# CITlabRostock/citlab-article-separation-new

Measured on AMD Instinct MI355X. Metric: newspaper pages/sec (ARU-Net seg + GNN relation) at 3000x4500 px, higher is better.
Workload: dtype f32s

## Files before the change

### citlab-article-separation-new_amd/csrc/aru_engine.hip

```cpp
#include <algorithm>
#include <cmath>
#include <cstdlib>
#include <memory>

#include "aru_kernels.h"
#include "res8_kernels.h"
#include "res8v_kernels.h"
#include "bf16_kernels.h"
#include "res8w_kernels.h"
#include "res8ws_kernels.h"
#include "level0_plan.h"
#include "launch_plan.h"
#include "convr_kernels.h"
#include "split_kernels.h"
#include "pyr_kernels.h"
#include "asep_common.h"
#include "aru_pack.h"

using namespace asep;

namespace {

struct Tensor {
    float* p = nullptr;
    int H = 0, W = 0, C = 0;
    bool bf = false;
    size_t count() const { return (size_t)H * W * C; }
    bf16_t* bp() const { return reinterpret_cast<bf16_t*>(p); }
};

struct PackedConv : ConvPlan {
    float* d_w = nullptr;
    float* d_b = nullptr;
    float* d_wino = nullptr;
    float* d_wv = nullptr;
    bf16_t* d_wb = nullptr;
    bf16_t* d_wb8 = nullptr;
    bf16_t* d_ws = nullptr;
    bf16_t* d_ws16 = nullptr;
};

struct DirectConv {
    int k = 0, cout = 0, cin = 1;
    float* d_w = nullptr;
    float* d_b = nullptr;
};

}

struct asep_aru {
    asep_aru_cfg cfg{};
    std::map<std::string, PackedConv> convs;
    struct ResB { int C = 0; bf16_t* d_w = nullptr; float* d_b = nullptr; };
    std::map<std::string, ResB> resb;
    std::map<std::string, float*> taps;
    bf16_t* d_r8b_down_w = nullptr;
    float* d_r8b_down_b = nullptr;
    bf16_t* d_r8b_up_w1 = nullptr;
    bf16_t* d_r8f_up_w1 = nullptr;
    bf16_t* d_r8f_down_w1 = nullptr;
    float* d_r8b_down_w1r = nullptr;
    bool use_res32 = true;
    int walk_mode = 1;
    bool use_deconvs = true;
    bool use_convr = true;
    unsigned char* d_zero_trash = nullptr;
    int fused_act = 0;
    bool use_walk = true;
    bf16_t* d_r8b_up_w = nullptr;
    float* d_r8b_up_b = nullptr;
    float* d_r8b_up_b1 = nullptr;
    DirectConv det_first, att_first;
    float* d_r8_down_wr = nullptr;
    float* d_r8_down_br = nullptr;
    float* d_r8_up_w1 = nullptr;
    float* d_r8_up_wr = nullptr;
    float* d_r8_up_br = nullptr;
    float* d_r8_up_b1 = nullptr;
    float* d_r8v_down_wr = nullptr;
    float* d_r8v_up_w1 = nullptr;
    float* d_r8v_up_wr = nullptr;
    bool r8_valu = true;
    bool use_split_walk = true;
    bf16_t* d_r8ws_down_w = nullptr;
    bf16_t* d_r8ws_up_w = nullptr;
    bf16_t* d_r8ws_up_w1 = nullptr;
    bool use_fused8 = true;
    bool fused8_wanted = true;
    bool fused8_var = false;
    float* d_att_head = nullptr;
    bf16_t* d_att_headb = nullptr;
    float* d_logit_w = nullptr;
    float* d_logit_b = nullptr;
    float* d_logit_wd = nullptr;
    float* d_stats = nullptr;
    const float* const* page_stats = nullptr;
    double* d_sums = nullptr;
    struct Lane {
        hipStream_t s = nullptr;
        bool own_stream = false;
        hipStream_t side = nullptr;
        hipEvent_t ev_fork = nullptr, ev_join = nullptr, ev_begin = nullptr, ev_done = nullptr;
        hipStream_t bside = nullptr;
        hipEvent_t ev_bfork = nullptr, ev_bjoin = nullptr;
        BufferPool pool;
        ~Lane() {
            if (ev_fork) (void)hipEventDestroy(ev_fork);
            if (ev_bfork) (void)hipEventDestroy(ev_bfork);
            if (ev_bjoin) (void)hipEventDestroy(ev_bjoin);
            if (ev_join) (void)hipEventDestroy(ev_join);
            if (ev_begin) (void)hipEventDestroy(ev_begin);
            if (ev_done) (void)hipEventDestroy(ev_done);
            if (side) (void)hipStreamDestroy(side);
            if (bside) (void)hipStreamDestroy(bside);
            if (own_stream && s) (void)hipStreamDestroy(s);
        }
    };
    std::vector<std::unique_ptr<Lane>> lanes;
    Lane* cur = nullptr;
    int last_nl = 0;
    bool lanes_forced = false;
    int num_lanes = 2;
    std::map<std::string, Tensor> endpoints;
    hipStream_t stream = nullptr;
    std::vector<void*> owned;

    struct ProfRec { int kid; double flops, bytes, xflops; hipEvent_t a, b; };
    int num_cus = 256;
    BufferPool host_stage;
    hipStream_t host_stream = nullptr;
    bool use_xcd_sched = true;
    std::map<std::string, const int32_t*> sched_cache;
    bool bf16 = false;
    bool split = false;
    bool use_c12 = true;
    bool fuse_pool = true;
    bool fuse_act = true;
    bool profiling = false;
    bool prof_detail = false;
    bool prof_in_situ = false;
    std::vector<std::string> prof_names;
    std::vector<ProfRec> prof_recs;
    std::vector<hipEvent_t> ev_pool;
    size_t ev_next = 0;

    ~asep_aru() {
        for (void* p : owned)
            if (p) (void)hipFree(p);
        for (hipEvent_t e : ev_pool) (void)hipEventDestroy(e);
        if (host_stream) (void)hipStreamDestroy(host_stream);
    }
    hipEvent_t next_event() {
        if (ev_next == ev_pool.size()) {
            hipEvent_t e;
            ASEP_HIP_CHECK_THROW(hipEventCreate(&e));
            ev_pool.push_back(e);
        }
        return ev_pool[ev_next++];
    }
    int prof_kid(const std::string& name) {
        for (size_t i = 0; i < prof_names.size(); ++i)
            if (prof_names[i] == name) return (int)i;
        prof_names.push_back(name);
        return (int)prof_names.size() - 1;
    }
    int feat(int l) const { return cfg.feat_root << l; }
// ... 414 lines not shown
        ProfScope ps(m, name, 0.0);
        ps.bytes = k.bytes;
        launch(a, dim3(k.units.total));
    });
}

TL run_pool(asep_aru* m, const TL& in, PoolKind kind) {
    TL out;
    for (const Tensor& t : in) {
        if (kind == POOL_CHANSUM) out.push_back(new_tensor(m, t.H, t.W, 1));
        else out.push_back(new_tensor(m, cdiv(t.H, 2), cdiv(t.W, 2), t.C));
    }
    stream_pass<PoolArgs>(m, in, kind == POOL_MAX ? "maxpool2_kernel" : (kind == POOL_AVG_C1 ? "avgpool2_c1_kernel" : (kind == POOL_AVG_C3 ? "avgpool2_cn_kernel<3>" : "chansum_kernel")), POOL_ITEMS,
        [&](PoolProb& p, size_t i, Chunk& k) {
            k.bytes += tbytes(in[i]) + tbytes(out[i]);
            p.in = in[i].p; p.out = out[i].p; p.H = in[i].H; p.W = in[i].W; p.Ho = out[i].H; p.Wo = out[i].W;
            return kind == POOL_MAX ? out[i].count() / 4 : (size_t)out[i].H * out[i].W;
        }, [&](const PoolArgs& a, dim3 grid) {
            if (kind == POOL_MAX) hipLaunchKernelGGL(maxpool2_kernel, grid, dim3(256), 0, m->stream, a);
            else if (kind == POOL_AVG_C1) hipLaunchKernelGGL(avgpool2_c1_kernel, grid, dim3(256), 0, m->stream, a);
            else if (kind == POOL_AVG_C3) launch_avgpool_c3(m, a, grid);
            else hipLaunchKernelGGL(chansum_kernel, grid, dim3(256), 0, m->stream, a);
        });
    return out;
}

int grid_1d(size_t n) { return (int)std::min<size_t>((n + 255) / 256, 256 * 8); }

std::string res8_what(bool up, const TL& l) {
    return (up ? "unet_up_0 (conv1[16->8]+3xconvR+add) " : "unet_down_0 (conv1+3xconvR+add+pool) ") + dims_of(l);
}

bool r8v_fits(const TL& l) {
    for (const Tensor& t : l)
        if ((size_t)t.H * t.W >= ((size_t)1 << 28)) return false;
    return true;
}

bool r8ws_fits(const Tensor& t) { return walk_region(t.H, t.W).fits; }
bool r8ws_on(asep_aru* m) { return m->split && m->use_split_walk && m->r8_valu && m->cfg.activation == 0 && m->d_r8ws_down_w; }
const int32_t* r8ws_frame_units(asep_aru* m, const Res8Args& a, const std::vector<bool>& walk, int* count) {
    std::string key = "f";
    for (int i = 0; i < a.nprob; ++i) key += ":" + std::to_string(a.p[i].H) + "x" + std::to_string(a.p[i].W) + (walk[i] ? "w" : "t");
    std::vector<int32_t> units;
    for (int i = 0; i < a.nprob; ++i) frame_units(a.p[i].H, a.p[i].W, a.p[i].tiles_x, a.p[i].tile_begin, walk[i], R8_OW, R8_OH * R8_NP, &units);
    *count = (int)units.size();
    auto it = m->sched_cache.find(key);
    if (it != m->sched_cache.end()) return it->second;
    if (units.empty()) return nullptr;
    const int32_t* d = put_table(m, units);
    if (d) m->sched_cache[key] = d;
    return d;
}

void run_res8ws(asep_aru* m, bool up, const Res8Args& a, const std::vector<bool>& walk, const std::string& what) {
    Res8WSArgs wa{};
    int n = 0, items = 0;
    double flops = 0, bytes = 0;
    long strip_rows = 0;
    for (int i = 0; i < a.nprob; ++i) {
        if (!walk[i]) continue;
        const Res8Prob& q = a.p[i];
        Res8WSProb& p = wa.p[n++];
        if (up) { p.skip = q.img; p.dec = q.in1; }
        else { p.img = q.img; p.stats = q.stats; p.pool = q.pool; }
        p.out = q.out;
        p.H = q.H; p.W = q.W;
        const WalkRegion r = walk_region(p.H, p.W);
        p.n_strips = r.n_strips;
        p.y_end = r.y_end;
        strip_rows += (long)r.n_strips * r.rows();
        flops += 2.0 * r.pixels() * (9.0 * (up ? 16 : 1) * 8 + 3 * 9.0 * 64);
        bytes += r.pixels() * ((up ? 64.0 : 4.0) + 32.0 + (p.pool ? 8.0 : 0.0));
    }
    if (!n) return;
    const int band = walk_band(strip_rows, m->num_cus, 4);
    for (int i = 0; i < n; ++i) {
        Res8WSProb& p = wa.p[i];
        p.band = band;
        p.tile_begin = items;
        items += walk_region(p.H, p.W).items(band);
    }
    wa.nprob = n;
    if (up) { wa.b1 = m->d_r8_up_b1; wa.w1s = (const u32x4*)m->d_r8ws_up_w1; wa.ws = (const u32x4*)m->d_r8ws_up_w; wa.bias = m->d_r8_up_br; }
    else { wa.b1 = m->det_first.d_b; wa.w1f = m->det_first.d_w; wa.ws = (const u32x4*)m->d_r8ws_down_w; wa.bias = m->d_r8_down_br; }
    int units = items;
    wa.xm = oneshot_map(m, items, &units);
    ProfScope ps(m, up ? "res8ws_kernel<true>" : "res8ws_kernel<false>", flops, what);
    ps.bytes = bytes;
    if (up) hipLaunchKernelGGL(res8ws_kernel<true>, dim3(units), dim3(64), 0, m->stream, wa);
    else hipLaunchKernelGGL(res8ws_kernel<false>, dim3(units), dim3(64), 0, m->stream, wa);
}

struct Res8Kernel { void (*fn)(const Res8Args); const char* name; };
Res8Kernel res8_kernel(bool up, bool valu, int actv) {
    static const Res8Kernel k[2][4] = {
        {{res8v_down_kernel<0>, "res8v_down_kernel<0>"}, {res8v_down_kernel<1>, "res8v_down_kernel<1>"}, {res8v_down_kernel<2>, "res8v_down_kernel<2>"},
         {res8_down_kernel<false>, "res8_down_kernel<false>"}},
        {{res8v_up_kernel<0>, "res8v_up_kernel<0>"}, {res8v_up_kernel<1>, "res8v_up_kernel<1>"}, {res8v_up_kernel<2>, "res8v_up_kernel<2>"},
         {res8_up_kernel<false>, "res8_up_kernel<false>"}}};
    return k[up][valu ? actv : 3];
}

void run_res8(asep_aru* m, bool up, const TL& in0, const TL* in1, const std::vector<const float*>& stats, bool want_pool, TL* d_out, TL* pool_out) {
    for (const Tensor& t : in0) {
        d_out->push_back(new_tensor(m, t.H, t.W, 8));
        if (want_pool) pool_out->push_back(new_tensor(m, cdiv(t.H, 2), cdiv(t.W, 2), 8));
    }
    const size_t lds = up ? R8_UP_LDS : R8_DOWN_LDS;
    const char* layer = up ? "unet_up_0" : "unet_down_0";
    for_chunks<Res8Args>(in0.size(), 0.0, [&](Res8Prob& p, size_t i, Chunk& k) {
        k.bytes += tbytes(in0[i]) + (up ? tbytes((*in1)[i]) : 0.0) + tbytes((*d_out)[i]) + (want_pool ? tbytes((*pool_out)[i]) : 0.0);
        p.img = in0[i].p; p.in1 = up ? (*in1)[i].p : nullptr; p.stats = stats.empty() ? nullptr : stats[i];
        p.out = (*d_out)[i].p; p.pool = want_pool ? (*pool_out)[i].p : nullptr;
        p.H = in0[i].H; p.W = in0[i].W;
        set_tiles(p, k.units.next_tiles(p.H, p.W, R8_OW, R8_OH * R8_NP));
        k.flops += 2.0 * in0[i].H * in0[i].W * (9.0 * (up ? 16 : 1) * 8 + 3 * 9.0 * 64);
    }, [&](Res8Args& a, const Chunk& c) {
        const int tiles = c.units.total;
        const double flops = c.flops, bytes = c.bytes;
        const TL sub = c.sub(in0);
        const bool valu = m->r8_valu && r8v_fits(sub);
        if (up) { a.w1 = valu ? m->d_r8v_up_w1 : m->d_r8_up_w1; a.b1 = m->d_r8_up_b1; }
        else { a.w1 = m->det_first.d_w; a.b1 = m->det_first.d_b; }
        a.wr = (const f32x4*)(up ? (valu ? m->d_r8v_up_wr : m->d_r8_up_wr) : (valu ? m->d_r8v_down_wr : m->d_r8_down_wr));
        a.br = up ? m->d_r8_up_br : m->d_r8_down_br;
        const int actv = m->cfg.activation;
        const Res8Kernel k = res8_kernel(up, valu, actv);
        a.sched = tile_schedule(m, a, std::min(tiles, m->num_cus), R8_OH * R8_NP);
        if (valu && r8ws_on(m) && (!up || m->d_r8ws_up_w1)) {
            std::vector<bool> walk(a.nprob);
            bool any = false;
            for (int i = 0; i < a.nprob; ++i) { walk[i] = r8ws_fits(sub[i]); any = any || walk[i]; }
            if (any) {
                int nu = 0;
                Res8Args f = a;
                f.sched = r8ws_frame_units(m, a, walk, &nu);
                if (!f.sched) { set_error("level-0 frame schedule: device allocation failed"); throw ArgError(); }
                f.total_tiles = nu;
                {
                    const double share = (double)nu / tiles;
                    ProfScope ps(m, k.name, flops * share, std::string(layer) + " frame " + dims_of(sub));
                    ps.bytes = bytes * share;
                    hipLaunchKernelGGL(k.fn, dim3(std::min(nu, m->num_cus)), dim3(R8_THREADS), lds, m->stream, f);
                }
                run_res8ws(m, up, a, walk, res8_what(up, sub));
                return;
            }
        }
        ProfScope ps(m, k.name, flops, res8_what(up, sub));
        ps.bytes = bytes;
        if (actv && !valu) { set_error("level-0 block of an elu / leaky graph: image too large for the vector-ALU kernel"); throw ArgError(); }
        hipLaunchKernelGGL(k.fn, dim3(std::min(tiles, m->num_cus)), dim3(R8_THREADS), lds, m->stream, a);
    });
}

void run_res8b_tiles(asep_aru* m, bool up, const TL& a0, const TL* a1, const std::vector<const float*>& stats, bool want_pool, const TL& outs, const TL* pool_out);

void run_res8w(asep_aru* m, bool up, const TL& in0, const TL* dec, const std::vector<const float*>& stats, const TL& outs, const TL* pools) {
    for (size_t c = 0; c < num_chunks(in0.size()); ++c) {
        const size_t b0 = chunk_begin(c), b1 = chunk_end(in0.size(), c);
        Res8WArgs wa{};
        Res8WBArgs ba{};
        double flops = 0, bytes = 0, wshare = 0;
        long strip_rows = 0;
        for (size_t i = b0; i < b1; ++i) {
// ... 915 lines not shown
    }
    if (fusedb && cfg->res_depth == 3)
        for (int l = 0; l < n; ++l) {
            const int f = cfg->feat_root << l;
            if (f != 8 && f != 16 && !(f == 32 && m->use_res32)) continue;
            for (const char* side : {"down", "up"}) {
                if (side[0] == 'u' && l == n - 1) continue;
                const std::string scope = std::string("aru_net/featMapG/unet_") + side + "_" + std::to_string(l);
                const ResbPack p = pack_resb(blob, scope, f);
                if (p.ok) m->resb[scope] = {f, m->put(p.w), m->put(p.b)};
            }
        }
    const Layer logit = find_layer(blob, "aru_net/logit/class");
    if (!has_shape(logit.w, 4, 4, cfg->feat_root, cfg->n_classes)) {
        set_error("weights: aru_net/logit/class/weights must be [4,4,%d,%d]", cfg->feat_root, cfg->n_classes);
        throw PackRefusal{ASEP_ERR_WEIGHTS};
    }
    m->d_logit_w = m->put(logit.w.data);
    m->d_logit_b = m->put(logit.b.data);
    if (cfg->n_classes == 2) m->d_logit_wd = m->put(pack_logit_diff(logit));
}

}

extern "C" {

asep_aru* asep_aru_load(const void* weight_blob, size_t nbytes, const asep_aru_cfg* cfg) {
    ASEP_GUARD_BEGIN
    if (!cfg || !weight_blob) { set_error("asep_aru_load: null argument"); return nullptr; }
    if (cfg->struct_size != (int32_t)sizeof(asep_aru_cfg)) {
        set_error("asep_aru_load: cfg.struct_size is %d, this library's asep_aru_cfg has %zu bytes (ABI version %d): the binding was "
                  "written against another include/asep_hip.h", cfg->struct_size, sizeof(asep_aru_cfg), ASEP_ABI_VERSION);
        return nullptr;
    }
    if (cfg->channels != 1 && cfg->channels != 3) { set_error("asep_aru_load: %d input channels: 1 (gray) and 3 (RGB) are supported", cfg->channels); return nullptr; }
    if (cfg->channels == 3 && cfg->use_attention) {
        set_error("asep_aru_load: 3-channel input needs a graph without attention (RU or U): the attention graph upsamples its attention map to the "
                  "input's shape with a one-channel filter (ARU_v1.py:115)");
        return nullptr;
    }
    if (cfg->compute_dtype < 0 || cfg->compute_dtype > 2) { set_error("asep_aru_load: compute_dtype %d unknown (0 = fp32, 1 = bf16 MFMA, 2 = fp32 with split bf16 products)", cfg->compute_dtype); return nullptr; }
    if (cfg->scale_space_num < 1 || cfg->res_depth < 1) { set_error("asep_aru_load: bad cfg"); return nullptr; }
    if (cfg->activation < 0 || cfg->activation > 2) { set_error("asep_aru_load: activation %d unknown (0 = relu, 1 = elu, 2 = leaky)", cfg->activation); return nullptr; }
    const bool variant = cfg->activation != 0 || cfg->plain_u != 0;
    if (cfg->plain_u && cfg->use_attention) { set_error("asep_aru_load: graph 'U' has no attention branch (ARU_v1.py:92-97)"); return nullptr; }
    if (cfg->inp4up && !cfg->input_pyramid) { set_error("asep_aru_load: inp4up is an option of the input-pyramid graph (RU_v2.py:143): set input_pyramid"); return nullptr; }
    if (cfg->input_pyramid && (cfg->use_attention || cfg->plain_u)) {
        set_error("asep_aru_load: the input-pyramid graph (RU_v2) is a residual U-Net without attention (RU_v2.py:56: useResidual=True, no attMapG): "
                  "use_attention and plain_u must be 0");
        return nullptr;
    }
    if (cfg->input_pyramid && cfg->compute_dtype == 1) {
        set_error("asep_aru_load: the input-pyramid graph (RU_v2) is served by the fp32 engines (compute_dtype 0 or 2): the bf16 engine's fused block "
                  "tails round conv1's result to bfloat16 before the pooled page's term could be added");
        return nullptr;
    }
    std::map<std::string, HostTensor> blob;
    if (!parse_blob(weight_blob, nbytes, blob)) return nullptr;
    std::map<std::string, std::vector<float>> taps;
    if (cfg->input_pyramid) {
        try {
            blob = split_pyramid_blob(blob, *cfg, taps);
        } catch (const PackRefusal&) {
            return nullptr;
        }
    }
    warn_ignored_switches();
    std::unique_ptr<asep_aru> m(new asep_aru());
    m->cfg = *cfg;
    m->bf16 = cfg->compute_dtype == 1;
    m->split = cfg->compute_dtype == 2;
    if (const char* e = getenv("ASEP_FUSE_POOL")) m->fuse_pool = atoi(e) != 0;
    if (const char* e = getenv("ASEP_FUSE_ACT")) m->fuse_act = atoi(e) != 0;
    if (const char* e = getenv("ASEP_C12")) m->use_c12 = atoi(e) != 0;
    if (const char* e = getenv("ASEP_FUSED8")) m->use_fused8 = atoi(e) != 0;
    m->fused8_wanted = m->use_fused8;
    if (variant) m->use_fused8 = false;
    if (const char* e = getenv("ASEP_R8_VALU")) m->r8_valu = atoi(e) != 0;
    m->fused8_var = variant && !cfg->plain_u && cfg->activation != 0 && m->fused8_wanted && m->r8_valu && m->fuse_act && !m->bf16;
    if (const char* e = getenv("ASEP_XCD_SCHED")) m->use_xcd_sched = atoi(e) != 0;
    if (const char* e = getenv("ASEP_BF_RES32")) m->use_res32 = atoi(e) != 0;
    if (const char* e = getenv("ASEP_BF_CONVR")) m->use_convr = atoi(e) != 0;
    if (const char* e = getenv("ASEP_SPLIT_DECONV")) m->use_deconvs = atoi(e) != 0;
    if (const char* e = getenv("ASEP_SPLIT_WALK")) m->use_split_walk = atoi(e) != 0;
    if (const char* e = getenv("ASEP_BF_WALK")) { m->walk_mode = atoi(e); m->use_walk = m->walk_mode != 0; }
    if (const char* e = getenv("ASEP_LANES")) { m->num_lanes = std::max(1, std::min(4, atoi(e))); m->lanes_forced = true; }
    for (int l = 0; l < m->num_lanes; ++l) {
        std::unique_ptr<asep_aru::Lane> L(new asep_aru::Lane());
        bool ok = hipStreamCreateWithFlags(&L->side, hipStreamNonBlocking) == hipSuccess &&
                  hipStreamCreateWithFlags(&L->bside, hipStreamNonBlocking) == hipSuccess &&
                  hipEventCreateWithFlags(&L->ev_fork, hipEventDisableTiming) == hipSuccess &&
                  hipEventCreateWithFlags(&L->ev_bfork, hipEventDisableTiming) == hipSuccess &&
                  hipEventCreateWithFlags(&L->ev_bjoin, hipEventDisableTiming) == hipSuccess &&
                  hipEventCreateWithFlags(&L->ev_join, hipEventDisableTiming) == hipSuccess &&
                  hipEventCreateWithFlags(&L->ev_begin, hipEventDisableTiming) == hipSuccess &&
                  hipEventCreateWithFlags(&L->ev_done, hipEventDisableTiming) == hipSuccess;
        if (ok && l > 0) { ok = hipStreamCreateWithFlags(&L->s, hipStreamNonBlocking) == hipSuccess; L->own_stream = ok; }
        if (!ok) { set_error("asep_aru_load: cannot create streams/events for lane %d", l); return nullptr; }
        m->lanes.push_back(std::move(L));
    }
    m->cur = m->lanes[0].get();
    for (const auto& t : taps) m->taps[t.first] = m->put(t.second);
    try {
        load_weights(m.get(), blob, variant);
    } catch (const PackRefusal&) {
        return nullptr;
    }
    {
        hipDeviceProp_t prop;
        int dev = 0;
        if (hipGetDevice(&dev) == hipSuccess && hipGetDeviceProperties(&prop, dev) == hipSuccess && prop.multiProcessorCount > 0)
            m->num_cus = prop.multiProcessorCount;
    }
    m->d_stats = m->alloc<float>(2);
    m->d_sums = m->alloc<double>(2);
    m->d_zero_trash = m->alloc<unsigned char>(8192);
    ASEP_HIP_CHECK_THROW(hipMemset(m->d_zero_trash, 0, 8192));
    return m.release();
    ASEP_GUARD_END_PTR
}

void asep_aru_free(asep_aru* m) { delete m; }

static int forward_lanes(asep_aru* m, int n_pages, const float* const* d_imgs, const int32_t* Hs, const int32_t* Ws, float* const* d_outs,
                         uint8_t* const* d_u8, uint8_t* const* d_mask, float threshold, hipStream_t stream) {
    m->endpoints.clear();
    const int by_pages = m->lanes_forced ? n_pages : n_pages / 4;
    const int nl = (m->profiling || n_pages < 2) ? 1 : std::max(1, std::min<int>((int)m->lanes.size(), by_pages));
    asep_aru::Lane& L0 = *m->lanes[0];
    L0.s = stream;
    if (nl != m->last_nl && n_pages > 1) {
        if (m->last_nl != 0)
            for (auto& Lp : m->lanes) Lp->pool.release();
        m->last_nl = nl;
    }
    if (nl == 1) return forward_impl(m, L0, 0, n_pages, d_imgs, Hs, Ws, d_outs, d_u8, d_mask, threshold);
    ASEP_HIP_CHECK(hipEventRecord(L0.ev_begin, stream));
    int page0 = 0;
    for (int l = 0; l < nl; ++l) {
        asep_aru::Lane& L = *m->lanes[l];
        const int cnt = n_pages / nl + (l < n_pages % nl ? 1 : 0);
        if (l > 0) ASEP_HIP_CHECK(hipStreamWaitEvent(L.s, L0.ev_begin, 0));
        int rc = forward_impl(m, L, page0, cnt, d_imgs + page0, Hs + page0, Ws + page0, d_outs + page0, d_u8 ? d_u8 + page0 : nullptr,
                              d_mask ? d_mask + page0 : nullptr, threshold);
        if (rc) return rc;
        if (l > 0) {
            ASEP_HIP_CHECK(hipEventRecord(L.ev_done, L.s));
            ASEP_HIP_CHECK(hipStreamWaitEvent(stream, L.ev_done, 0));
        }
        page0 += cnt;
    }
    m->stream = stream;
    return ASEP_OK;
}

int asep_aru_forward_dev(asep_aru* m, const float* d_img, int H, int W, float* d_out, uint8_t* d_out_u8,
                         uint8_t* d_out_mask, float threshold, void* stream) {
    ASEP_GUARD_BEGIN
    if (!m || !d_img || !d_out || H < 1 || W < 1) { set_error("asep_aru_forward_dev: bad argument"); return ASEP_ERR_ARG; }
    const int32_t h1 = H, w1 = W;
    return forward_lanes(m, 1, &d_img, &h1, &w1, &d_out, d_out_u8 ? &d_out_u8 : nullptr, d_out_mask ? &d_out_mask : nullptr,
                         threshold, (hipStream_t)stream);
    ASEP_GUARD_END
}

int asep_aru_forward_batch_dev(asep_aru* m, int n_pages, const float* const* d_imgs, int H, int W, float* const* d_outs,
                               uint8_t* const* d_out_u8, uint8_t* const* d_out_mask, float threshold, void* stream) {
// ... 180 lines not shown
```

### citlab-article-separation-new_amd/csrc/res8ws_kernels.h

```cpp
#pragma once
#include "res8w_kernels.h"
#include "split_kernels.h"

namespace asep {

struct Res8WSProb {
    const float* skip;
    const float* dec;
    const float* img;
    const float* stats;
    float* out;
    float* pool;
    int H, W;
    int n_strips;
    int band;
    int y_end;
    int tile_begin;
};
struct Res8WSArgs {
    Res8WSProb p[MAXP];
    int nprob;
    const float* b1;
    const u32x4* w1s;
    const float* w1f;
    const u32x4* ws;
    const float* bias;
    XcdMap xm;
};

__device__ __forceinline__ void r8ws_mm6(const u32x4 (&w)[3], const u32x4 (&xa)[3], const u32x4 (&xb)[3], f32x4& ca, f32x4& cb) {
    ca = mfma_bf16_k32(w[2], xa[0], ca); cb = mfma_bf16_k32(w[2], xb[0], cb);
    ca = mfma_bf16_k32(w[0], xa[2], ca); cb = mfma_bf16_k32(w[0], xb[2], cb);
    ca = mfma_bf16_k32(w[1], xa[1], ca); cb = mfma_bf16_k32(w[1], xb[1], cb);
    ca = mfma_bf16_k32(w[1], xa[0], ca); cb = mfma_bf16_k32(w[1], xb[0], cb);
    ca = mfma_bf16_k32(w[0], xa[1], ca); cb = mfma_bf16_k32(w[0], xb[1], cb);
    ca = mfma_bf16_k32(w[0], xa[0], ca); cb = mfma_bf16_k32(w[0], xb[0], cb);
}
__device__ __forceinline__ void r8ws_split4(f32x4 v, u32x2& h, u32x2& m, u32x2& l) {
    unsigned h0, m0, l0, h1, m1, l1;
    split3_pair(v.x, v.y, h0, m0, l0);
    split3_pair(v.z, v.w, h1, m1, l1);
    h = u32x2{h0, h1}; m = u32x2{m0, m1}; l = u32x2{l0, l1};
}

template <bool UP>
__global__ __launch_bounds__(64, 1) void res8ws_kernel(const Res8WSArgs a) {
    constexpr int TW = R8W_TW;
    constexpr int W0 = TW + 6, W1 = TW + 4, W2 = TW + 2;
    constexpr int NR = 4, NT = 16;
    constexpr int PL0 = W0 * 16, PL1 = W1 * 16, PL2 = W2 * 16;
    constexpr int IMB = UP ? 0 : 4 * 32 * 4;
    constexpr int R0_OFF = IMB, R1_OFF = R0_OFF + NR * 3 * PL0, R2_OFF = R1_OFF + NR * 3 * PL1, TC_OFF = R2_OFF + NR * 3 * PL2,
                  TRASH = TC_OFF + NT * TW * 32, LDSB = TRASH + 16;
    static_assert(LDSB <= 30 * 1024, "four waves per CU with room to spare");
    __shared__ __attribute__((aligned(16))) unsigned char lds[LDSB];

    const int lane = threadIdx.x;
    const int j = lane & 15, kk = lane >> 4, e = kk >> 1, ch = (kk & 1) * 4;
    const int isB = kk & 1;
    const int c = 2 * j + e;
    const int item = sched_tile(a.xm);
    if (item < 0) return;
    const int pi = prob_of_tile(a, item);
    const Res8WSProb& P = a.p[pi];
    const int li = item - P.tile_begin;
    const int bi = li / P.n_strips, si = li - bi * P.n_strips;
    const int x0 = R8W_X0 + TW * si;
    const int Ya = R8W_Y0 + bi * P.band;
    const int nb = min(P.band, P.y_end - Ya);
    const int W = P.W;

    constexpr int NF1 = UP ? 18 : 0, NFW = 27;
    u32x4 wf[NFW], w1[UP ? NF1 : 1];
    {
        const u32x4* wl = a.ws + lane;
#pragma unroll
        for (int i = 0; i < NFW; ++i) asm volatile("global_load_dwordx4 %0, %1, off" : "=a"(wf[i]) : "v"(wl + i * 64) : "memory");
        if constexpr (UP) {
            const u32x4* w1l = a.w1s + lane;
#pragma unroll
            for (int i = 0; i < NF1; ++i) asm volatile("global_load_dwordx4 %0, %1, off" : "=a"(w1[i]) : "v"(w1l + i * 64) : "memory");
        }
        asm volatile("s_waitcnt vmcnt(0)" ::: "memory");
#pragma unroll
        for (int i = 0; i < NFW; ++i) asm volatile("" : "+a"(wf[i]));
        if constexpr (UP) {
#pragma unroll
            for (int i = 0; i < NF1; ++i) asm volatile("" : "+a"(w1[i]));
        }
    }
    auto wpart = [&](int s, int ky, u32x4 (&o)[3]) {
#pragma unroll
        for (int p = 0; p < 3; ++p) o[p] = wf[(s * 3 + ky) * 3 + p];
    };
    const f32x4 bias1 = *reinterpret_cast<const f32x4*>(a.b1 + ch);
    f32x4 biasw[3];
#pragma unroll
    for (int t = 0; t < 3; ++t) biasw[t] = *reinterpret_cast<const f32x4*>(a.bias + 8 * t + ch);

    const int gxw = min(x0 - 4 + 2 * j + kk, W - 1);
    const float* __restrict__ skp = P.skip;
    const float* __restrict__ dcp = P.dec;
    auto in_row = [&](const float* __restrict__ src, int gy, f32x4& lo, f32x4& hi) {
        const float* q = src + ((size_t)gy * (size_t)W + (size_t)gxw) * 8;
        lo = *reinterpret_cast<const f32x4*>(q);
        hi = *reinterpret_cast<const f32x4*>(q + 4);
    };
    float mean = 0.f, inv = 1.f;
    if constexpr (!UP) {
        if (P.stats) { mean = P.stats[0]; inv = P.stats[1]; }
    }
    const float* __restrict__ imp = P.img;
    const size_t ioff0 = (size_t)(Ya - 4 + (lane >> 5)) * (size_t)W + (size_t)(x0 - 4 + (lane & 31));
    auto iload = [&](int p) { return imp[ioff0 + (size_t)p * 2 * (size_t)W]; };
    float* const iring = reinterpret_cast<float*>(lds);
    auto istore = [&](float v, int p) { iring[(p & 1) * 64 + lane] = (v - mean) * inv; };
    float w1v[UP ? 1 : 36];
    if constexpr (!UP) {
#pragma unroll
        for (int t = 0; t < 9; ++t)
#pragma unroll
            for (int o = 0; o < 4; ++o) w1v[t * 4 + o] = a.w1f[t * 8 + ch + o];
    }

    const int p_last = nb / 2 + 3;
    u32x4 cin[2][2][3] = {};
    f32x4 nxt[2][2][2];
    float inx = 0.f;
    if constexpr (UP) {
#pragma unroll
        for (int r = 0; r < 2; ++r) {
            f32x4 lo, hi;
            in_row(skp, Ya - 4 + r, lo, hi);
            split3_x8(lo, hi, cin[r][0][0], cin[r][0][1], cin[r][0][2]);
            in_row(dcp, Ya - 4 + r, lo, hi);
            split3_x8(lo, hi, cin[r][1][0], cin[r][1][1], cin[r][1][2]);
            in_row(skp, Ya - 2 + r, nxt[r][0][0], nxt[r][0][1]);
            in_row(dcp, Ya - 2 + r, nxt[r][1][0], nxt[r][1][1]);
        }
    } else {
        istore(iload(0), 0);
        inx = iload(1);
    }

    const int lcol = r8w_swz(2 * j + kk) * 16;
    auto whole = [&](u32x2 pa, u32x2 pb) {
        const auto s0 = __builtin_amdgcn_permlane16_swap(pa.x, pb.x, false, false);
        const auto s1 = __builtin_amdgcn_permlane16_swap(pa.y, pb.y, false, false);
        return u32x4{s0[0], s1[0], s0[1], s1[1]};
    };
    const int cs = r8w_swz(c) * 16;
    const bool v0 = j < W0 / 2, v1 = j < W1 / 2, v2 = j < W2 / 2;
    const bool tvalid = c >= 3 && c < 3 + TW;
    const int tcol = (tvalid ? c - 3 : 0) * 32 + ch * 4;
    const int trd = min(c, TW - 1) * 32 + ch * 4;
    const bool ost = j < TW / 2;
    float* __restrict__ const outp = P.out;
    float* __restrict__ const poolp = P.pool;
    const size_t Wp = (size_t)((W + 1) >> 1);

    auto store_parts = [&](f32x4 ra, f32x4 rb, int roff, int pl, bool valid, int rowa, int rowb) {
        u32x2 ha, ma, la, hb, mb, lb;
        r8ws_split4(relu4i(ra), ha, ma, la);
        r8ws_split4(relu4i(rb), hb, mb, lb);
        const u32x4 ph = whole(ha, hb), pm = whole(ma, mb), pl_ = whole(la, lb);
        const int rr = isB ? rowb : rowa;
        const int base = valid ? roff + rr * 3 * pl + cs : TRASH;
        const int step = valid ? pl : 0;
        *reinterpret_cast<u32x4*>(lds + base) = ph;
        *reinterpret_cast<u32x4*>(lds + base + step) = pm;
        *reinterpret_cast<u32x4*>(lds + base + 2 * step) = pl_;
    };
    auto ring_read = [&](int roff, int pl, int rr, u32x4 (&o)[3]) {
#pragma unroll
        for (int p = 0; p < 3; ++p) o[p] = *reinterpret_cast<const u32x4*>(lds + roff + (rr * 3 + p) * pl + lcol);
    };

    const int K = nb / 2 + 6;
#pragma unroll 1
    for (int k = 0; k < K; ++k) {
        const int i4 = (2 * k) & (NR - 1), i16 = (2 * k) & (NT - 1);
        const bool do_c1 = k < nb / 2 + 3, do_s1 = k >= 2 && k < nb / 2 + 4, do_s2 = k >= 4 && k < nb / 2 + 5, do_s3 = k >= 6;

        if (do_s3) {
            u32x4 q[4][3];
#pragma unroll
            for (int r = 0; r < 4; ++r) ring_read(R2_OFF, PL2, (i4 + r - 9) & (NR - 1), q[r]);
            const f32x4 t0 = *reinterpret_cast<const f32x4*>(lds + TC_OFF + ((i16 - 8) & (NT - 1)) * TW * 32 + trd);
            const f32x4 t1 = *reinterpret_cast<const f32x4*>(lds + TC_OFF + ((i16 - 7) & (NT - 1)) * TW * 32 + trd);
            f32x4 va = biasw[2], vb = biasw[2];
#pragma unroll
            for (int ky = 0; ky < 3; ++ky) {
                u32x4 w[3];
                wpart(2, ky, w);
                r8ws_mm6(w, q[ky], q[ky + 1], va, vb);
            }
            va = relu4i(va + t0);
            vb = relu4i(vb + t1);
            const int oy = Ya - 12 + 2 * k;
            if (ost) {
                float* o = outp + ((size_t)oy * (size_t)W + (size_t)(x0 + c)) * 8 + ch;
                *reinterpret_cast<f32x4*>(o) = va;
                *reinterpret_cast<f32x4*>(o + (size_t)W * 8) = vb;
            }
            if constexpr (!UP) {
                if (poolp) {
                    const f32x4 mv = f32x4{fmaxf(va.x, vb.x), fmaxf(va.y, vb.y), fmaxf(va.z, vb.z), fmaxf(va.w, vb.w)};
                    float pm[4];
#pragma unroll
                    for (int i = 0; i < 4; ++i) {
                        const unsigned u = __float_as_uint(mv[i]);
                        const auto s = __builtin_amdgcn_permlane32_swap(u, u, false, false);
                        pm[i] = fmaxf(__uint_as_float(s[0]), __uint_as_float(s[1]));
                    }
                    if (ost && e == 0) {
                        float* po = poolp + ((size_t)(oy >> 1) * Wp + (size_t)((x0 >> 1) + j)) * 8 + ch;
                        *reinterpret_cast<f32x4*>(po) = f32x4{pm[0], pm[1], pm[2], pm[3]};
                    }
                }
            }
        }
        if (do_s2) {
            u32x4 q[4][3];
#pragma unroll
            for (int r = 0; r < 4; ++r) ring_read(R1_OFF, PL1, (i4 + r - 6) & (NR - 1), q[r]);
            f32x4 ra = biasw[1], rb = biasw[1];
#pragma unroll
            for (int ky = 0; ky < 3; ++ky) {
                u32x4 w[3];
                wpart(1, ky, w);
                r8ws_mm6(w, q[ky], q[ky + 1], ra, rb);
            }
            store_parts(ra, rb, R2_OFF, PL2, v2, (i4 - 5) & (NR - 1), (i4 - 4) & (NR - 1));
        }
        if (do_s1) {
            u32x4 q[4][3];
#pragma unroll
            for (int r = 0; r < 4; ++r) ring_read(R0_OFF, PL0, (i4 + r - 3) & (NR - 1), q[r]);
            f32x4 ra = biasw[0], rb = biasw[0];
#pragma unroll
            for (int ky = 0; ky < 3; ++ky) {
                u32x4 w[3];
                wpart(0, ky, w);
                r8ws_mm6(w, q[ky], q[ky + 1], ra, rb);
            }
            store_parts(ra, rb, R1_OFF, PL1, v1, (i4 - 2) & (NR - 1), (i4 - 1) & (NR - 1));
        }
        if (do_c1) {
            f32x4 ra = bias1, rb = bias1;
            if constexpr (UP) {
                u32x4 x2[2][2][3];
#pragma unroll
                for (int r = 0; r < 2; ++r)
#pragma unroll
                    for (int s = 0; s < 2; ++s) split3_x8(nxt[r][s][0], nxt[r][s][1], x2[r][s][0], x2[r][s][1], x2[r][s][2]);
                if (k + 2 <= p_last) {
#pragma unroll
                    for (int r = 0; r < 2; ++r) {
                        in_row(skp, Ya + 2 * k + r, nxt[r][0][0], nxt[r][0][1]);
                        in_row(dcp, Ya + 2 * k + r, nxt[r][1][0], nxt[r][1][1]);
                    }
                }
#pragma unroll
                for (int ky = 0; ky < 3; ++ky)
#pragma unroll
                    for (int s = 0; s < 2; ++s) {
                        u32x4 w[3];
#pragma unroll
                        for (int p = 0; p < 3; ++p) w[p] = w1[(ky * 2 + s) * 3 + p];
                        u32x4 xa[3], xb[3];
#pragma unroll
                        for (int p = 0; p < 3; ++p) {
                            xa[p] = ky == 0 ? cin[0][s][p] : (ky == 1 ? cin[1][s][p] : x2[0][s][p]);
                            xb[p] = ky == 0 ? cin[1][s][p] : (ky == 1 ? x2[0][s][p] : x2[1][s][p]);
                        }
                        r8ws_mm6(w, xa, xb, ra, rb);
                    }
#pragma unroll
                for (int r = 0; r < 2; ++r)
#pragma unroll
                    for (int s = 0; s < 2; ++s)
#pragma unroll
                        for (int p = 0; p < 3; ++p) cin[r][s][p] = x2[r][s][p];
            } else {
                istore(inx, k + 1);
                if (k + 2 <= p_last) inx = iload(k + 2);
                const int cb = min(c, 29);
#pragma unroll
                for (int ky = 0; ky < 3; ++ky)
#pragma unroll
                    for (int kx = 0; kx < 3; ++kx) {
                        const float va = iring[((2 * k + ky) & 3) * 32 + cb + kx], vb = iring[((2 * k + 1 + ky) & 3) * 32 + cb + kx];
#pragma unroll
                        for (int o = 0; o < 4; ++o) {
                            ra[o] = fmaf(va, w1v[(ky * 3 + kx) * 4 + o], ra[o]);
                            rb[o] = fmaf(vb, w1v[(ky * 3 + kx) * 4 + o], rb[o]);
                        }
                    }
            }
            if (tvalid) {
                *reinterpret_cast<f32x4*>(lds + TC_OFF + ((i16 + 1) & (NT - 1)) * TW * 32 + tcol) = ra;
                *reinterpret_cast<f32x4*>(lds + TC_OFF + ((i16 + 2) & (NT - 1)) * TW * 32 + tcol) = rb;
            }
            store_parts(ra, rb, R0_OFF, PL0, v0, (i4 + 1) & (NR - 1), (i4 + 2) & (NR - 1));
        }
    }
}

}
```

Baseline: 152.1.

## Add unrolled steady-state loop to split-walk res8 kernel with deferred output stores

Restructures the res8ws strip-walk loop into a branch-free steady-state body, unrolled by two with compile-time ring indices. Boundary conditions become clamped loads and trash-slot LDS writes so the middle iterations run without predication. For the up variant, global output stores are deferred to the end of each iteration so they overlap the MFMA work. The down kernel's launch bounds now allow two waves per CU. This adds code size and register pressure, and keeps the old path selectable via ASEP_SPLIT_WALK=2.

```diff
diff --git a/citlab-article-separation-new_amd/csrc/aru_engine.hip b/citlab-article-separation-new_amd/csrc/aru_engine.hip
--- a/citlab-article-separation-new_amd/csrc/aru_engine.hip
+++ b/citlab-article-separation-new_amd/csrc/aru_engine.hip
@@ -82,6 +82,7 @@
     float* d_r8v_up_wr = nullptr;
     bool r8_valu = true;
     bool use_split_walk = true;
+    bool split_walk_steady = true;
     bf16_t* d_r8ws_down_w = nullptr;
     bf16_t* d_r8ws_up_w = nullptr;
     bf16_t* d_r8ws_up_w1 = nullptr;
@@ -662,6 +663,7 @@
         items += walk_region(p.H, p.W).items(band);
     }
     wa.nprob = n;
+    wa.steady = m->split_walk_steady ? 1 : 0;
     if (up) { wa.b1 = m->d_r8_up_b1; wa.w1s = (const u32x4*)m->d_r8ws_up_w1; wa.ws = (const u32x4*)m->d_r8ws_up_w; wa.bias = m->d_r8_up_br; }
     else { wa.b1 = m->det_first.d_b; wa.w1f = m->det_first.d_w; wa.ws = (const u32x4*)m->d_r8ws_down_w; wa.bias = m->d_r8_down_br; }
     int units = items;
@@ -1743,7 +1745,7 @@
     if (const char* e = getenv("ASEP_BF_RES32")) m->use_res32 = atoi(e) != 0;
     if (const char* e = getenv("ASEP_BF_CONVR")) m->use_convr = atoi(e) != 0;
     if (const char* e = getenv("ASEP_SPLIT_DECONV")) m->use_deconvs = atoi(e) != 0;
-    if (const char* e = getenv("ASEP_SPLIT_WALK")) m->use_split_walk = atoi(e) != 0;
+    if (const char* e = getenv("ASEP_SPLIT_WALK")) { m->use_split_walk = atoi(e) != 0; m->split_walk_steady = atoi(e) != 2; }
     if (const char* e = getenv("ASEP_BF_WALK")) { m->walk_mode = atoi(e); m->use_walk = m->walk_mode != 0; }
     if (const char* e = getenv("ASEP_LANES")) { m->num_lanes = std::max(1, std::min(4, atoi(e))); m->lanes_forced = true; }
     for (int l = 0; l < m->num_lanes; ++l) {
diff --git a/citlab-article-separation-new_amd/csrc/res8ws_kernels.h b/citlab-article-separation-new_amd/csrc/res8ws_kernels.h
--- a/citlab-article-separation-new_amd/csrc/res8ws_kernels.h
+++ b/citlab-article-separation-new_amd/csrc/res8ws_kernels.h
@@ -25,6 +25,7 @@
     const float* w1f;
     const u32x4* ws;
     const float* bias;
+    int steady;
     XcdMap xm;
 };
 
@@ -44,7 +45,7 @@
 }
 
 template <bool UP>
-__global__ __launch_bounds__(64, 1) void res8ws_kernel(const Res8WSArgs a) {
+__global__ __launch_bounds__(64, UP ? 1 : 2) void res8ws_kernel(const Res8WSArgs a) {
     constexpr int TW = R8W_TW;
     constexpr int W0 = TW + 6, W1 = TW + 4, W2 = TW + 2;
     constexpr int NR = 4, NT = 16;
@@ -113,8 +114,10 @@
     const float* __restrict__ imp = P.img;
     const size_t ioff0 = (size_t)(Ya - 4 + (lane >> 5)) * (size_t)W + (size_t)(x0 - 4 + (lane & 31));
     auto iload = [&](int p) { return imp[ioff0 + (size_t)p * 2 * (size_t)W]; };
+    const int irow0 = Ya - 4 + (lane >> 5), icol = x0 - 4 + (lane & 31), Hm1 = P.H - 1;
+    auto iload_c = [&](int p) { return imp[(size_t)min(irow0 + 2 * p, Hm1) * (size_t)W + (size_t)icol]; };
     float* const iring = reinterpret_cast<float*>(lds);
-    auto istore = [&](float v, int p) { iring[(p & 1) * 64 + lane] = (v - mean) * inv; };
+    auto istore = [&](float v, int slot) { iring[slot * 64 + lane] = (v - mean) * inv; };
     float w1v[UP ? 1 : 36];
     if constexpr (!UP) {
 #pragma unroll
@@ -176,27 +179,19 @@
         for (int p = 0; p < 3; ++p) o[p] = *reinterpret_cast<const u32x4*>(lds + roff + (rr * 3 + p) * pl + lcol);
     };
 
-    const int K = nb / 2 + 6;
-#pragma unroll 1
-    for (int k = 0; k < K; ++k) {
-        const int i4 = (2 * k) & (NR - 1), i16 = (2 * k) & (NT - 1);
-        const bool do_c1 = k < nb / 2 + 3, do_s1 = k >= 2 && k < nb / 2 + 4, do_s2 = k >= 4 && k < nb / 2 + 5, do_s3 = k >= 6;
-
-        if (do_s3) {
-            u32x4 q[4][3];
-#pragma unroll
-            for (int r = 0; r < 4; ++r) ring_read(R2_OFF, PL2, (i4 + r - 9) & (NR - 1), q[r]);
-            const f32x4 t0 = *reinterpret_cast<const f32x4*>(lds + TC_OFF + ((i16 - 8) & (NT - 1)) * TW * 32 + trd);
-            const f32x4 t1 = *reinterpret_cast<const f32x4*>(lds + TC_OFF + ((i16 - 7) & (NT - 1)) * TW * 32 + trd);
-            f32x4 va = biasw[2], vb = biasw[2];
-#pragma unroll
-            for (int ky = 0; ky < 3; ++ky) {
-                u32x4 w[3];
-                wpart(2, ky, w);
-                r8ws_mm6(w, q[ky], q[ky + 1], va, vb);
-            }
-            va = relu4i(va + t0);
-            vb = relu4i(vb + t1);
+    constexpr int TROW = TW * 32;
+    auto iteration = [&](auto phase_c, const int k, const int trb, const int twb, const int twn) {
+        constexpr int PH = decltype(phase_c)::value;
+        constexpr bool ST = PH >= 0;
+        constexpr bool DEFER = ST && UP;
+        const int i4 = ST ? 2 * PH : (2 * k) & (NR - 1), i16 = (2 * k) & (NT - 1);
+        const bool do_c1 = ST || k < nb / 2 + 3, do_s1 = ST || (k >= 2 && k < nb / 2 + 4), do_s2 = ST || (k >= 4 && k < nb / 2 + 5), do_s3 = ST || k >= 6;
+        const int tr0 = ST ? trb + 2 * PH * TROW : ((i16 - 8) & (NT - 1)) * TROW, tr1 = ST ? tr0 + TROW : ((i16 - 7) & (NT - 1)) * TROW;
+        const int tw0 = ST ? twb + (2 * PH + 1) * TROW : ((i16 + 1) & (NT - 1)) * TROW;
+        const int tw1 = ST ? (PH == 0 ? twb + 2 * TROW : twn) : ((i16 + 2) & (NT - 1)) * TROW;
+
+        f32x4 va = biasw[2], vb = biasw[2];
+        auto out_stores = [&]() {
             const int oy = Ya - 12 + 2 * k;
             if (ost) {
                 float* o = outp + ((size_t)oy * (size_t)W + (size_t)(x0 + c)) * 8 + ch;
@@ -219,6 +214,22 @@
                     }
                 }
             }
+        };
+        if (do_s3) {
+            u32x4 q[4][3];
+#pragma unroll
+            for (int r = 0; r < 4; ++r) ring_read(R2_OFF, PL2, (i4 + r - 9) & (NR - 1), q[r]);
+            const f32x4 t0 = *reinterpret_cast<const f32x4*>(lds + TC_OFF + tr0 + trd);
+            const f32x4 t1 = *reinterpret_cast<const f32x4*>(lds + TC_OFF + tr1 + trd);
+#pragma unroll
+            for (int ky = 0; ky < 3; ++ky) {
+                u32x4 w[3];
+                wpart(2, ky, w);
+                r8ws_mm6(w, q[ky], q[ky + 1], va, vb);
+            }
+            va = relu4i(va + t0);
+            vb = relu4i(vb + t1);
+            if constexpr (!DEFER) out_stores();
         }
         if (do_s2) {
             u32x4 q[4][3];
@@ -254,11 +265,12 @@
                 for (int r = 0; r < 2; ++r)
 #pragma unroll
                     for (int s = 0; s < 2; ++s) split3_x8(nxt[r][s][0], nxt[r][s][1], x2[r][s][0], x2[r][s][1], x2[r][s][2]);
-                if (k + 2 <= p_last) {
+                if (ST || k + 2 <= p_last) {
 #pragma unroll
                     for (int r = 0; r < 2; ++r) {
-                        in_row(skp, Ya + 2 * k + r, nxt[r][0][0], nxt[r][0][1]);
-                        in_row(dcp, Ya + 2 * k + r, nxt[r][1][0], nxt[r][1][1]);
+                        const int gy = ST ? min(Ya + 2 * k + r, P.H - 1) : Ya + 2 * k + r;
+                        in_row(skp, gy, nxt[r][0][0], nxt[r][0][1]);
+                        in_row(dcp, gy, nxt[r][1][0], nxt[r][1][1]);
                     }
                 }
 #pragma unroll
@@ -283,14 +295,15 @@
 #pragma unroll
                         for (int p = 0; p < 3; ++p) cin[r][s][p] = x2[r][s][p];
             } else {
-                istore(inx, k + 1);
-                if (k + 2 <= p_last) inx = iload(k + 2);
+                istore(inx, ST ? (PH + 1) & 1 : (k + 1) & 1);
+                if constexpr (ST) inx = iload_c(k + 2);
+                else if (k + 2 <= p_last) inx = iload(k + 2);
                 const int cb = min(c, 29);
 #pragma unroll
                 for (int ky = 0; ky < 3; ++ky)
 #pragma unroll
                     for (int kx = 0; kx < 3; ++kx) {
-                        const float va = iring[((2 * k + ky) & 3) * 32 + cb + kx], vb = iring[((2 * k + 1 + ky) & 3) * 32 + cb + kx];
+                        const float va = iring[((i4 + ky) & 3) * 32 + cb + kx], vb = iring[((i4 + 1 + ky) & 3) * 32 + cb + kx];
 #pragma unroll
                         for (int o = 0; o < 4; ++o) {
                             ra[o] = fmaf(va, w1v[(ky * 3 + kx) * 4 + o], ra[o]);
@@ -298,12 +311,32 @@
                         }
                     }
             }
-            if (tvalid) {
-                *reinterpret_cast<f32x4*>(lds + TC_OFF + ((i16 + 1) & (NT - 1)) * TW * 32 + tcol) = ra;
-                *reinterpret_cast<f32x4*>(lds + TC_OFF + ((i16 + 2) & (NT - 1)) * TW * 32 + tcol) = rb;
+            if constexpr (ST) {
+                *reinterpret_cast<f32x4*>(lds + (tvalid ? TC_OFF + tw0 + tcol : TRASH)) = ra;
+                *reinterpret_cast<f32x4*>(lds + (tvalid ? TC_OFF + tw1 + tcol : TRASH)) = rb;
+            } else if (tvalid) {
+                *reinterpret_cast<f32x4*>(lds + TC_OFF + tw0 + tcol) = ra;
+                *reinterpret_cast<f32x4*>(lds + TC_OFF + tw1 + tcol) = rb;
             }
             store_parts(ra, rb, R0_OFF, PL0, v0, (i4 + 1) & (NR - 1), (i4 + 2) & (NR - 1));
         }
+        if constexpr (DEFER) out_stores();
+    };
+
+    const int K = nb / 2 + 6;
+    const int ks_end = a.steady ? nb / 2 + 3 : 0;
+#pragma unroll 1
+    for (int k = 0; k < K;) {
+        if (k >= 6 && !(k & 1) && k + 2 <= ks_end) {
+            const int tb = (2 * k) & (NT - 1);
+            const int trb = (tb ^ 8) * TROW, twb = tb * TROW, twn = ((tb + 4) & (NT - 1)) * TROW;
+            iteration(ic<0>{}, k, trb, twb, twn);
+            iteration(ic<1>{}, k + 1, trb, twb, twn);
+            k += 2;
+        } else {
+            iteration(ic<-1>{}, k, 0, 0, 0);
+            ++k;
+        }
     }
 }
 
```

After: 153.5 (median of 6 runs). About the same (+0.9%).
